# numz/ComfyUI-SeedVR2_VideoUpscaler

Measured on AMD Instinct MI355X. Metric: upscaled frames/sec (720p->4K, SeedVR2-3B), higher is better.
Workload: dtype bf16; 1 GPU; cfg3: SeedVR2-3B 32-frame 720p->4K clip (padded to 33 = 4n+1 for encode + DiT, 32 decoded), VAE tiled 1024/128; vae_tiled=True, parallelism=dp1, weights=random-init SeedVR2-3B + video_vae_v3 architecture (seeded)

## Files before the change

comfyui-seedvr2_videoupscaler_amd/csrc/svr_conv_sub.hip:

```cpp
#include "svr_common.h"
#include "../../include/seedvr2_hip.h"
#include <type_traits>

namespace svr {

constexpr int CS_TY = 16, CS_TX = 32, CS_HX = CS_TX + 1, CS_HY = CS_TY + 1;
constexpr int CS_NT = 256;
constexpr int CS_ROWS = CS_HX * CS_HY;
constexpr int CS_PIECES = (CS_ROWS * 4 + CS_NT - 1) / CS_NT;
constexpr int CS_ABUF = CS_PIECES * CS_NT * 16;
constexpr int CS_NBUF = 4;
constexpr int CS_EP_PITCH = 528;
constexpr int CS_EP_BYTES = 4 * 32 * CS_EP_PITCH;
constexpr int CS_LDS = CS_NBUF * CS_ABUF;
static_assert(CS_PIECES == 9 && CS_EP_BYTES <= CS_LDS, "piece schedule / epilogue parking");

template <int OFF> SVR_DEVICE void cs_rd2(bf16x8 (&r)[2], unsigned a0) {
    const unsigned a1 = a0 ^ 32u;
    asm volatile("ds_read_b128 %0, %2 offset:%4\n\tds_read_b128 %1, %3 offset:%4"
                 : "=&v"(r[0]), "=&v"(r[1]) : "v"(a0), "v"(a1), "n"(OFF) : "memory");
}
template <int N> SVR_DEVICE void cs_wait_rows(bf16x8 (&a)[2]) {
    asm volatile("s_waitcnt lgkmcnt(%2)" : "+v"(a[0]), "+v"(a[1]) : "n"(N));
    __builtin_amdgcn_sched_barrier(0);
}
template <int N> SVR_DEVICE void cs_wait_rows(bf16x8 (&a)[2], bf16x8 (&b)[2]) {
    asm volatile("s_waitcnt lgkmcnt(%4)" : "+v"(a[0]), "+v"(a[1]), "+v"(b[0]), "+v"(b[1]) : "n"(N));
    __builtin_amdgcn_sched_barrier(0);
}
template <int N> SVR_DEVICE void cs_wait_rows(bf16x8 (&a)[2], bf16x8 (&b)[2], bf16x8 (&c)[2], bf16x8 (&d)[2], bf16x8 (&e)[2]) {
    asm volatile("s_waitcnt lgkmcnt(%10)"
                 : "+v"(a[0]), "+v"(a[1]), "+v"(b[0]), "+v"(b[1]), "+v"(c[0]), "+v"(c[1]), "+v"(d[0]), "+v"(d[1]), "+v"(e[0]), "+v"(e[1])
                 : "n"(N));
    __builtin_amdgcn_sched_barrier(0);
}
template <int N> SVR_DEVICE void cs_wait_w(bf16x8 (&w)[2][2]) {
    asm volatile("s_waitcnt vmcnt(%4)" : "+v"(w[0][0]), "+v"(w[0][1]), "+v"(w[1][0]), "+v"(w[1][1]) : "n"(N));
    __builtin_amdgcn_sched_barrier(0);
}

__global__ __launch_bounds__(CS_NT, 1) void conv_sub_kernel(const svr_gemm_args a, const int band_rows) {
    constexpr int MTW = 8, NTW = 2, NT = CS_NT;
    extern __shared__ __attribute__((aligned(16))) char smem[];
    typedef __attribute__((ext_vector_type(16))) float f32x16_t;
    const svr_conv_geom& g = a.conv;
    const int tid = threadIdx.x;
    const int lane = tid & 63;
    const int wave = __builtin_amdgcn_readfirstlane(tid >> 6);
    const int wm = wave >> 1, wn = wave & 1;

    const int tiles_x = (g.W + CS_TX - 1) / CS_TX;
    const int tiles_y = (g.H + CS_TY - 1) / CS_TY;
    const int tiles_n = a.N / 128;
    int tl;
    {
        const int nwg = gridDim.x, bid = blockIdx.x;
        const int xcd = bid & 7, j = bid >> 3, q = nwg >> 3, r = nwg & 7;
        tl = (xcd < r ? xcd * (q + 1) : r * (q + 1) + (xcd - r) * q) + j;
    }
    const bool quad = a.phase.enabled && a.phase.quad != 0;
    int qp = 0;
    if (quad) { qp = tl & 3; tl >>= 2; }
    const int ph_py = quad ? (qp >> 1) : a.phase.py, ph_px = quad ? (qp & 1) : a.phase.px;
    const int pad_h = quad ? 1 - ph_py : g.ph, pad_w = quad ? 1 - ph_px : g.pw;
    const void* const w_frag = quad ? a.phase.W_frag4[qp] : a.W_frag;
    const float* const bias_p = quad ? a.phase.bias4[qp] : a.bias;
    const float* const bias_border_p = quad ? a.phase.bias_border4[qp] : a.phase.bias_border;
    const int tn = tl % tiles_n;
    int rr = tl / tiles_n;
    const int tx = rr % tiles_x; rr /= tiles_x;
    int ty, to;
    if (band_rows > 0 && band_rows < tiles_y) {
        const int per_band = band_rows * g.To;
        const int b = rr / per_band;
        const int rows_b = min(band_rows, tiles_y - b * band_rows);
        const int r2 = rr - b * per_band;
        to = r2 / rows_b;
        ty = b * band_rows + (r2 - to * rows_b);
    } else {
        ty = rr % tiles_y;
        to = rr / tiles_y;
    }
    const int y0 = ty * CS_TY, x0 = tx * CS_TX, n0 = tn * 128;

    const int cpk = g.Cin / 32;
    const int nA = g.kt * cpk;
    const int P = nA * 4;
    const int64_t frame_bytes = (int64_t)g.H * g.W * g.Cin * 2;
    const int srow = tid >> 2, spos = tid & 3;
    uint32_t poff[CS_PIECES];
    uint32_t akeys = 0;
#pragma unroll
    for (int q = 0; q < CS_PIECES; ++q) {
        const int row = q * (NT / 4) + srow;
        const int hy = row / CS_HX, hx = row - hy * CS_HX;
        const int y = y0 - pad_h + hy, x = x0 - pad_w + hx;
        const bool ok = (row < CS_ROWS) & ((unsigned)y < (unsigned)g.H) & ((unsigned)x < (unsigned)g.W);
        poff[q] = ok ? (uint32_t)(y * g.W + x) : 0xffffffffu;
        akeys |= (uint32_t)(spos ^ ((hx >> 2) & 3)) << (2 * q);
    }
    char* const wave_dst = smem + wave * 1024;
    auto frame_ptr = [&](int s) -> const char* {
        if (s >= nA) return nullptr;
        const int dt = s / cpk;
        const int c0 = (s - dt * cpk) * 32;
        int f = to + dt - g.pt;
        const char* basep = (const char*)a.A;
        if (f < 0) {
            if (g.halo != nullptr) { basep = (const char*)g.halo; f += g.halo_frames; }
            else f = 0;
        }
        return basep + (int64_t)f * frame_bytes + c0 * 2;
    };
    auto stage = [&](auto qc, const char* fptr, int buf) {
        constexpr int Q = decltype(qc)::value;
        const int ck = (akeys >> (2 * Q)) & 3;
        const char* src = (poff[Q] == 0xffffffffu || fptr == nullptr) ? (const char*)g.zeros
                                                                      : fptr + ((int64_t)poff[Q] * g.Cin + ck * 8) * 2;
        glds16(src, wave_dst + buf * CS_ABUF + Q * (NT * 16));
    };
    auto stage_all = [&](const char* fptr, int buf) {
        stage(std::integral_constant<int, 0>{}, fptr, buf); stage(std::integral_constant<int, 1>{}, fptr, buf);
        stage(std::integral_constant<int, 2>{}, fptr, buf); stage(std::integral_constant<int, 3>{}, fptr, buf);
        stage(std::integral_constant<int, 4>{}, fptr, buf); stage(std::integral_constant<int, 5>{}, fptr, buf);
        stage(std::integral_constant<int, 6>{}, fptr, buf); stage(std::integral_constant<int, 7>{}, fptr, buf);
        stage(std::integral_constant<int, 8>{}, fptr, buf);
    };

    const int l31 = lane & 31, hi = lane >> 5;
    const unsigned lds0 = (unsigned)(uintptr_t)(__attribute__((address_space(3))) char*)smem;
    unsigned fa[2];
#pragma unroll
    for (int dx = 0; dx < 2; ++dx)
        fa[dx] = lds0 + (unsigned)((wm * MTW * CS_HX + l31) * 64 + ((hi ^ (((dx + l31) >> 2) & 3)) << 4));

    f32x16_t acc[MTW][NTW];
#pragma unroll
    for (int y = 0; y < MTW; ++y)
#pragma unroll
        for (int z = 0; z < NTW; ++z)
#pragma unroll
            for (int e = 0; e < 16; ++e) acc[y][z][e] = 0.f;
    bf16x8 a0[2], a1[2], a2[2], a3[2], a4[2], a5[2], a6[2], a7[2], a8[2];
    bf16x8 w0[NTW][2], w1[NTW][2], w2[NTW][2], w3[NTW][2];

    const int64_t nstride = (int64_t)P * 2048;
    const char* wp0 = (const char*)w_frag + (int64_t)(n0 / 32 + wn * 2) * nstride;
    const char* wp1 = wp0 + nstride;
    const int voff = lane * 16;
    auto wload = [&](bf16x8 (&w)[NTW][2], int k) {
        auto uniform_ptr = [](const char* p) {
            const uint64_t u = (uint64_t)p;
            const uint32_t lo = __builtin_amdgcn_readfirstlane((uint32_t)u), hi_ = __builtin_amdgcn_readfirstlane((uint32_t)(u >> 32));
            return (const char*)(((uint64_t)hi_ << 32) | lo);
        };
        const char* p0 = uniform_ptr(wp0 + (int64_t)min(k, P - 1) * 2048);
        const char* p1 = uniform_ptr(wp1 + (int64_t)min(k, P - 1) * 2048);
        asm volatile("global_load_dwordx4 %0, %1, %2" : "=v"(w[0][0]) : "v"(voff), "s"(p0) : "memory");
        asm volatile("global_load_dwordx4 %0, %1, %2 offset:1024" : "=v"(w[0][1]) : "v"(voff), "s"(p0) : "memory");
        asm volatile("global_load_dwordx4 %0, %1, %2" : "=v"(w[1][0]) : "v"(voff), "s"(p1) : "memory");
        asm volatile("global_load_dwordx4 %0, %1, %2 offset:1024" : "=v"(w[1][1]) : "v"(voff), "s"(p1) : "memory");
    };

#define CS_RD(ROW, R, DXV, BUFOFF) cs_rd2<((R) * CS_HX + (DXV)) * 64>(ROW, fa[DXV] + (BUFOFF))
#define CS_MM(W, KS, ROW, MT, NTI) \
    acc[MT][NTI] = __builtin_amdgcn_mfma_f32_32x32x16_bf16(W[NTI][KS], ROW[KS], acc[MT][NTI], 0, 0, 0)
#define CS_MM8(W, RA, MA, RB, MB) \
    CS_MM(W, 0, RA, MA, 0); CS_MM(W, 0, RA, MA, 1); CS_MM(W, 0, RB, MB, 0); CS_MM(W, 0, RB, MB, 1); \
    CS_MM(W, 1, RA, MA, 0); CS_MM(W, 1, RA, MA, 1); CS_MM(W, 1, RB, MB, 0); CS_MM(W, 1, RB, MB, 1)

    auto interval = [&](auto jc, int s, const char* fstage, bf16x8 (&wc)[NTW][2], bf16x8 (&wn_)[NTW][2]) {
        constexpr int J = decltype(jc)::value;
        constexpr int DX = J >> 1, DY = J & 1;
        constexpr int NPC[4] = {0, 0, 5, 4};
        constexpr int NV = 4 + NPC[(J + 3) & 3] + NPC[(J + 2) & 3];
        const int k = s * 4 + J;
        const unsigned cur = (unsigned)((s & 3) * CS_ABUF), nxt = (unsigned)(((s + 1) & 3) * CS_ABUF);
        const int sbuf = (s + 3) & 3;
        constexpr int NDX = DX ^ 1;
        const unsigned nb = DX == 0 ? cur : nxt;
        if constexpr (DY == 0) {
            CS_RD(a8, 8, DX, cur);
            cs_wait_rows<8>(a0, a1, a2, a3, a4);
            cs_wait_w<NV>(wc);
            CS_MM8(wc, a0, 0, a1, 1);
            __builtin_amdgcn_sched_barrier(0);
            CS_RD(a0, 0, NDX, nb);
            wload(wn_, k + 2);
            __builtin_amdgcn_sched_barrier(0);
            CS_MM8(wc, a2, 2, a3, 3);
            __builtin_amdgcn_sched_barrier(0);
            if constexpr (J == 2) {
                stage(std::integral_constant<int, 0>{}, fstage, sbuf); stage(std::integral_constant<int, 1>{}, fstage, sbuf);
                stage(std::integral_constant<int, 2>{}, fstage, sbuf);
            }
            cs_wait_rows<8>(a4, a5);
            CS_MM8(wc, a4, 4, a5, 5);
            __builtin_amdgcn_sched_barrier(0);
            if constexpr (J == 2) { stage(std::integral_constant<int, 3>{}, fstage, sbuf); stage(std::integral_constant<int, 4>{}, fstage, sbuf); }
            cs_wait_rows<4>(a6, a7);
            CS_MM8(wc, a6, 6, a7, 7);
            __builtin_amdgcn_sched_barrier(0);
        } else {
            cs_wait_w<NV>(wc);
            CS_MM8(wc, a1, 0, a2, 1);
            __builtin_amdgcn_sched_barrier(0);
            CS_RD(a1, 1, NDX, nb); CS_RD(a2, 2, NDX, nb);
            wload(wn_, k + 2);
            __builtin_amdgcn_sched_barrier(0);
            CS_MM8(wc, a3, 2, a4, 3);
            __builtin_amdgcn_sched_barrier(0);
            CS_RD(a3, 3, NDX, nb); CS_RD(a4, 4, NDX, nb);
            if constexpr (J == 3) { stage(std::integral_constant<int, 5>{}, fstage, sbuf); stage(std::integral_constant<int, 6>{}, fstage, sbuf); }
            __builtin_amdgcn_sched_barrier(0);
            CS_MM8(wc, a5, 4, a6, 5);
            __builtin_amdgcn_sched_barrier(0);
            CS_RD(a5, 5, NDX, nb); CS_RD(a6, 6, NDX, nb);
            if constexpr (J == 3) { stage(std::integral_constant<int, 7>{}, fstage, sbuf); stage(std::integral_constant<int, 8>{}, fstage, sbuf); }
            cs_wait_rows<14>(a8);
            CS_MM8(wc, a7, 6, a8, 7);
            __builtin_amdgcn_sched_barrier(0);
            CS_RD(a7, 7, NDX, nb);
            if constexpr (J == 1) {
                __builtin_amdgcn_s_barrier();
                __builtin_amdgcn_sched_barrier(0);
            }
        }
    };

    stage_all(frame_ptr(0), 0);
    stage_all(frame_ptr(1), 1);
    stage_all(frame_ptr(2), 2);
    wload(w0, 0);
    wload(w1, 1);
    __builtin_amdgcn_sched_barrier(0);
#pragma unroll
    for (int y = 0; y < MTW; ++y)
#pragma unroll
        for (int z = 0; z < NTW; ++z) asm volatile("" : "+a"(acc[y][z]));
    asm volatile("s_waitcnt vmcnt(0)" ::: "memory");
    __builtin_amdgcn_s_barrier();
    __builtin_amdgcn_sched_barrier(0);
    CS_RD(a0, 0, 0, 0u); CS_RD(a1, 1, 0, 0u); CS_RD(a2, 2, 0, 0u); CS_RD(a3, 3, 0, 0u);
    CS_RD(a4, 4, 0, 0u); CS_RD(a5, 5, 0, 0u); CS_RD(a6, 6, 0, 0u); CS_RD(a7, 7, 0, 0u);

    for (int s = 0; s < nA; ++s) {
        const char* fs = frame_ptr(s + 3);
        interval(std::integral_constant<int, 0>{}, s, fs, w0, w2);
        interval(std::integral_constant<int, 1>{}, s, fs, w1, w3);
        interval(std::integral_constant<int, 2>{}, s, fs, w2, w0);
        interval(std::integral_constant<int, 3>{}, s, fs, w3, w1);
    }
    asm volatile("s_waitcnt vmcnt(0) lgkmcnt(0)" ::: "memory");
    __builtin_amdgcn_sched_barrier(0);
    __syncthreads();
#undef CS_RD
#undef CS_MM
#undef CS_MM8

    const int hi4 = hi * 4;
    const int n = n0 + (tid & 15) * 8;
    f32x4 bias_lo = {0.f, 0.f, 0.f, 0.f}, bias_hi = {0.f, 0.f, 0.f, 0.f};
    if (bias_p) {
        bias_lo = *(const f32x4*)(bias_p + n);
        bias_hi = *(const f32x4*)(bias_p + n + 4);
    }
    const int py = a.phase.enabled ? ph_py : 0, px = a.phase.enabled ? ph_px : 0;
    const int up = a.phase.enabled ? 2 : 1, ts = a.phase.enabled ? a.phase.t_stride : 1;
    const int yb = py ? g.H - 1 : 0, xb = px ? g.W - 1 : 0;
    const float* btab = a.phase.enabled ? bias_border_p : nullptr;
    double gs0 = 0.0, gq0 = 0.0, gs1 = 0.0, gq1 = 0.0;
    auto ep_body = [&](auto o32c) {
    constexpr int OKIND = decltype(o32c)::value;
    constexpr bool O32 = OKIND == SVR_STORE_FP32;
#pragma unroll
    for (int pass = 0; pass < MTW / 2; ++pass) {
        __builtin_amdgcn_sched_barrier(0);
#pragma unroll
        for (int j = 0; j < 2; ++j) {
            char* row = smem + ((wm * 2 + j) * 32 + l31) * CS_EP_PITCH;
#pragma unroll
            for (int nt = 0; nt < NTW; ++nt) {
                const f32x16_t v = acc[2 * pass + j][nt];
#pragma unroll
                for (int gq = 0; gq < 4; ++gq) {
                    const f32x4 o = {v[4 * gq], v[4 * gq + 1], v[4 * gq + 2], v[4 * gq + 3]};
                    *(f32x4*)(row + (wn * 64 + nt * 32 + 8 * gq + hi4) * 4) = o;
                }
            }
        }
        lds_barrier();
#pragma unroll
        for (int half = 0; half < 2; ++half) {
            f32x4 lo[4], hi_[4];
            int64_t off[4];
            bool ok[4];
            int border[4];
#pragma unroll
            for (int it = 0; it < 4; ++it) {
                const int vox = ((half * 4 + it) * NT + tid) >> 4;
                const int r = vox >> 5;
                const int y = y0 + (r >> 1) * MTW + 2 * pass + (r & 1), x = x0 + (vox & 31);
                ok[it] = y < g.H && x < g.W;
                const int yc = min(y, g.H - 1), xc = min(x, g.W - 1);
                border[it] = (yc == yb ? 1 : 0) | (xc == xb ? 2 : 0);
                off[it] = (((int64_t)to * ts * (up * g.H) + up * yc + py) * (up * g.W) + up * xc + px) * a.N + n;
                lo[it] = *(const f32x4*)(smem + vox * CS_EP_PITCH + (tid & 15) * 32);
                hi_[it] = *(const f32x4*)(smem + vox * CS_EP_PITCH + (tid & 15) * 32 + 16);
            }
#pragma unroll
            for (int it = 0; it < 4; ++it) {
                f32x4 bl = bias_lo, bh = bias_hi;
                if (btab != nullptr && border[it] != 0) {
                    const float* bb = btab + (int64_t)(border[it] - 1) * a.N + n;
                    bl = *(const f32x4*)bb;
                    bh = *(const f32x4*)(bb + 4);
                }
                const float f[8] = {lo[it][0] + bl[0], lo[it][1] + bl[1], lo[it][2] + bl[2], lo[it][3] + bl[3],
                                    hi_[it][0] + bh[0], hi_[it][1] + bh[1], hi_[it][2] + bh[2], hi_[it][3] + bh[3]};
                float r[8];
                if constexpr (O32) {
                    if (ok[it]) {
                        float* cp = (float*)a.C + off[it];
                        *(float4*)cp = make_float4(f[0], f[1], f[2], f[3]);
                        *(float4*)(cp + 4) = make_float4(f[4], f[5], f[6], f[7]);
                    }
#pragma unroll
                    for (int e = 0; e < 8; ++e) r[e] = f[e];
                } else {
                    const uint4 pk = OKIND == SVR_STORE_H16 ? pack8h(f) : pack8(f);
                    if (ok[it]) *(uint4*)((bf16_t*)a.C + off[it]) = pk;
                    if constexpr (OKIND == SVR_STORE_H16) unpack8h(pk, r); else unpack8(pk, r);
                }
                if (a.gn_partial != nullptr && ok[it]) {
                    gn_accumulate4(gs0, gq0, r[0], r[1], r[2], r[3]);
                    gn_accumulate4(gs1, gq1, r[4], r[5], r[6], r[7]);
                }
            }
        }
        if (pass + 1 < MTW / 2) lds_barrier();
    }
    };
    if (a.out_f32 == SVR_STORE_FP32) ep_body(std::integral_constant<int, SVR_STORE_FP32>{});
    else if (a.out_f32 == SVR_STORE_H16) ep_body(std::integral_constant<int, SVR_STORE_H16>{});
    else ep_body(std::integral_constant<int, SVR_STORE_BF16>{});
    if (a.gn_partial) {
        __syncthreads();
        double4* red = (double4*)smem;
        double2* qsum = (double2*)(smem + NT * 32);
        red[tid] = make_double4(gs0, gq0, gs1, gq1);
        __syncthreads();
        if (tid < 32) {
            const int c = tid >> 1, h = tid & 1;
            double s_ = 0.0, q_ = 0.0;
            for (int j = 0; j < NT / 16; ++j) {
                const double4 v = red[(j << 4) | c];
                s_ += h ? v.z : v.x;
                q_ += h ? v.w : v.y;
            }
            qsum[tid] = make_double2(s_, q_);
        }
        __syncthreads();
        const int qpg = (a.N / a.gn_groups) >> 2;
        if (tid < 32 / qpg) {
            double s_ = 0.0, q_ = 0.0;
            for (int i = 0; i < qpg; ++i) { s_ += qsum[tid * qpg + i].x; q_ += qsum[tid * qpg + i].y; }
            const int nblk = tiles_y * tiles_x;
            const int per_frame = a.phase.enabled ? 4 * nblk : nblk;
            const int slot = (a.phase.enabled ? (py * 2 + px) * nblk : 0) + ty * tiles_x + tx;
            ((double2*)a.gn_partial)[((int64_t)to * ts * per_frame + slot) * a.gn_groups + (n0 >> 2) / qpg + tid] = make_double2(s_, q_);
        }
    }
}

int g_conv_sub = 1;

static bool conv_sub_gn_ok(const svr_gemm_args& a) {
    const int cpg = a.gn_groups > 0 ? a.N / a.gn_groups : 0;
    return cpg >= 4 && !(cpg & 3) && a.N % a.gn_groups == 0 && 128 % cpg == 0;
}

static bool conv_sub_eligible(const svr_gemm_args& a) {
    const svr_conv_geom& g = a.conv;
    const bool quad = a.phase.enabled && a.phase.quad != 0;
    bool ptrs = true;
    if (quad) {
        for (int p = 0; p < 4; ++p)
            ptrs = ptrs && a.phase.W_frag4[p] != nullptr && (!a.phase.bias4[p] || ((uintptr_t)a.phase.bias4[p] % 16) == 0) &&
                   (!a.phase.bias_border4[p] || ((uintptr_t)a.phase.bias_border4[p] % 16) == 0);
    } else {
        ptrs = a.W_frag != nullptr && (unsigned)g.ph <= 1u && (unsigned)g.pw <= 1u && (!a.bias || ((uintptr_t)a.bias % 16) == 0) &&
               (!a.phase.bias_border || ((uintptr_t)a.phase.bias_border % 16) == 0);
    }
    return g_conv_sub && g.enabled && ptrs && g.kh == 2 && g.kw == 2 && g.sh == 1 && g.sw == 1 && g.st == 1 &&
           g.Ho == g.H && g.Wo == g.W && g.Cin % 32 == 0 && g.kt >= 1 && g.kt <= 3 &&
           g.To == g.T + g.pt - g.kt + 1 && !a.ps.enabled && a.epilogue == SVR_EPI_BIAS && !a.resid && !a.gate &&
           (!a.gn_partial || conv_sub_gn_ok(a)) && (a.N % 128) == 0 && (a.phase.enabled || (a.ldc == a.N)) &&
           (int64_t)g.H * g.W * g.Cin * 2 < (int64_t)1 << 32 && ((uintptr_t)a.C % 16) == 0;
}

static int conv_sub_gn_blocks(const svr_gemm_args& a) {
    if (!conv_sub_eligible(a) || !conv_sub_gn_ok(a)) return 0;
    const int nblk = ((a.conv.H + CS_TY - 1) / CS_TY) * ((a.conv.W + CS_TX - 1) / CS_TX);
    return a.phase.enabled ? 4 * nblk : nblk;
}

static int launch_conv_sub(const svr_gemm_args& a, hipStream_t s) {
    const svr_conv_geom& g = a.conv;
    const int tiles = g.To * ((g.H + CS_TY - 1) / CS_TY) * ((g.W + CS_TX - 1) / CS_TX) * (a.N / 128) *
                      (a.phase.enabled && a.phase.quad ? 4 : 1);
    static uint64_t lds_attr_done = 0;
    {
        const int e = set_max_dynamic_lds((const void*)conv_sub_kernel, 160 * 1024, lds_attr_done);
        if (e != 0) return e;
    }
    hipLaunchKernelGGL(conv_sub_kernel, dim3(tiles), dim3(CS_NT), CS_LDS, s, a, g_conv_band);
    return (int)hipGetLastError();
}

__global__ __launch_bounds__(256) void conv_pack_frag_taps_kernel(const bf16_t* __restrict__ W, uint4* __restrict__ out, int N, int K,
                                                                  int kt, int kh, int kw, int Cin) {
    const int cpk = Cin / 32, taps = kh * kw, P = kt * cpk * taps;
    const int64_t idx = (int64_t)blockIdx.x * 256 + threadIdx.x;
    if (idx >= (int64_t)(N / 32) * P * 128) return;
    const int lane = (int)(idx & 63), ks = (int)((idx >> 6) & 1);
    const int kk = (int)((idx >> 7) % P), n32 = (int)((idx >> 7) / P);
    const int s = kk / taps, J = kk - s * taps;
    const int dt = s / cpk, cs = s - dt * cpk, dy = J % kh, dx = J / kh;
    const int nn = n32 * 32 + (lane & 31), c = cs * 32 + ks * 16 + (lane >> 5) * 8;
    out[idx] = *(const uint4*)(W + (int64_t)nn * K + ((dt * kh + dy) * kw + dx) * Cin + c);
}

}
```

Measured before the change: 3.703 frames/s.

## Switch conv_sub inner MFMA from 32x32x16 to 16x16x32 bf16 tiles

Replaces each 32x32x16 MFMA with four 16x16x32 MFMAs and rewrites the fragment layout to match: the LDS row addressing and swizzle, the weight-load lane offsets, the accumulator shape, and the epilogue scatter into LDS. The likely aim is the shorter issue latency of the 16x16 instruction and finer interleaving with the LDS reads. In exchange it issues four times as many MFMA instructions for the same work and changes the LDS bank-access pattern.

Measured after the change: 3.728 frames/s (median of 6 runs). No clear change (+0.7%).

```diff
diff --git a/comfyui-seedvr2_videoupscaler_amd/csrc/svr_conv_sub.hip b/comfyui-seedvr2_videoupscaler_amd/csrc/svr_conv_sub.hip
--- a/comfyui-seedvr2_videoupscaler_amd/csrc/svr_conv_sub.hip
+++ b/comfyui-seedvr2_videoupscaler_amd/csrc/svr_conv_sub.hip
@@ -16,9 +16,15 @@
 static_assert(CS_PIECES == 9 && CS_EP_BYTES <= CS_LDS, "piece schedule / epilogue parking");
 
 template <int OFF> SVR_DEVICE void cs_rd2(bf16x8 (&r)[2], unsigned a0) {
-    const unsigned a1 = a0 ^ 32u;
-    asm volatile("ds_read_b128 %0, %2 offset:%4\n\tds_read_b128 %1, %3 offset:%4"
-                 : "=&v"(r[0]), "=&v"(r[1]) : "v"(a0), "v"(a1), "n"(OFF) : "memory");
+    static_assert(OFF >= 0 && OFF + 1024 + 16 <= 65536, "ds_read_b128 offset field");
+    asm volatile("ds_read_b128 %0, %2 offset:%3\n\tds_read_b128 %1, %2 offset:%4"
+                 : "=&v"(r[0]), "=&v"(r[1]) : "v"(a0), "n"(OFF), "n"(OFF + 1024) : "memory");
+}
+SVR_DEVICE void cs_mm4(f32x4 (&c)[2][2], const bf16x8 (&w)[2], const bf16x8 (&r)[2]) {
+    c[0][0] = __builtin_amdgcn_mfma_f32_16x16x32_bf16(w[0], r[0], c[0][0], 0, 0, 0);
+    c[0][1] = __builtin_amdgcn_mfma_f32_16x16x32_bf16(w[1], r[0], c[0][1], 0, 0, 0);
+    c[1][0] = __builtin_amdgcn_mfma_f32_16x16x32_bf16(w[0], r[1], c[1][0], 0, 0, 0);
+    c[1][1] = __builtin_amdgcn_mfma_f32_16x16x32_bf16(w[1], r[1], c[1][1], 0, 0, 0);
 }
 template <int N> SVR_DEVICE void cs_wait_rows(bf16x8 (&a)[2]) {
     asm volatile("s_waitcnt lgkmcnt(%2)" : "+v"(a[0]), "+v"(a[1]) : "n"(N));
@@ -42,7 +48,6 @@
 __global__ __launch_bounds__(CS_NT, 1) void conv_sub_kernel(const svr_gemm_args a, const int band_rows) {
     constexpr int MTW = 8, NTW = 2, NT = CS_NT;
     extern __shared__ __attribute__((aligned(16))) char smem[];
-    typedef __attribute__((ext_vector_type(16))) float f32x16_t;
     const svr_conv_geom& g = a.conv;
     const int tid = threadIdx.x;
     const int lane = tid & 63;
@@ -127,27 +132,27 @@
         stage(std::integral_constant<int, 8>{}, fptr, buf);
     };
 
-    const int l31 = lane & 31, hi = lane >> 5;
+    const int l15 = lane & 15, kq = lane >> 4;
     const unsigned lds0 = (unsigned)(uintptr_t)(__attribute__((address_space(3))) char*)smem;
     unsigned fa[2];
 #pragma unroll
     for (int dx = 0; dx < 2; ++dx)
-        fa[dx] = lds0 + (unsigned)((wm * MTW * CS_HX + l31) * 64 + ((hi ^ (((dx + l31) >> 2) & 3)) << 4));
-
-    f32x16_t acc[MTW][NTW];
+        fa[dx] = lds0 + (unsigned)((wm * MTW * CS_HX + l15) * 64 + ((kq ^ (((dx + l15) >> 2) & 3)) << 4));
+
+    f32x4 acc[MTW][NTW][2][2];
 #pragma unroll
     for (int y = 0; y < MTW; ++y)
 #pragma unroll
         for (int z = 0; z < NTW; ++z)
 #pragma unroll
-            for (int e = 0; e < 16; ++e) acc[y][z][e] = 0.f;
+            for (int e = 0; e < 16; ++e) acc[y][z][e >> 3][(e >> 2) & 1][e & 3] = 0.f;
     bf16x8 a0[2], a1[2], a2[2], a3[2], a4[2], a5[2], a6[2], a7[2], a8[2];
     bf16x8 w0[NTW][2], w1[NTW][2], w2[NTW][2], w3[NTW][2];
 
     const int64_t nstride = (int64_t)P * 2048;
     const char* wp0 = (const char*)w_frag + (int64_t)(n0 / 32 + wn * 2) * nstride;
     const char* wp1 = wp0 + nstride;
-    const int voff = lane * 16;
+    const int voff = kq * 512 + l15 * 16;
     auto wload = [&](bf16x8 (&w)[NTW][2], int k) {
         auto uniform_ptr = [](const char* p) {
             const uint64_t u = (uint64_t)p;
@@ -157,17 +162,14 @@
         const char* p0 = uniform_ptr(wp0 + (int64_t)min(k, P - 1) * 2048);
         const char* p1 = uniform_ptr(wp1 + (int64_t)min(k, P - 1) * 2048);
         asm volatile("global_load_dwordx4 %0, %1, %2" : "=v"(w[0][0]) : "v"(voff), "s"(p0) : "memory");
-        asm volatile("global_load_dwordx4 %0, %1, %2 offset:1024" : "=v"(w[0][1]) : "v"(voff), "s"(p0) : "memory");
+        asm volatile("global_load_dwordx4 %0, %1, %2 offset:256" : "=v"(w[0][1]) : "v"(voff), "s"(p0) : "memory");
         asm volatile("global_load_dwordx4 %0, %1, %2" : "=v"(w[1][0]) : "v"(voff), "s"(p1) : "memory");
-        asm volatile("global_load_dwordx4 %0, %1, %2 offset:1024" : "=v"(w[1][1]) : "v"(voff), "s"(p1) : "memory");
+        asm volatile("global_load_dwordx4 %0, %1, %2 offset:256" : "=v"(w[1][1]) : "v"(voff), "s"(p1) : "memory");
     };
 
 #define CS_RD(ROW, R, DXV, BUFOFF) cs_rd2<((R) * CS_HX + (DXV)) * 64>(ROW, fa[DXV] + (BUFOFF))
-#define CS_MM(W, KS, ROW, MT, NTI) \
-    acc[MT][NTI] = __builtin_amdgcn_mfma_f32_32x32x16_bf16(W[NTI][KS], ROW[KS], acc[MT][NTI], 0, 0, 0)
 #define CS_MM8(W, RA, MA, RB, MB) \
-    CS_MM(W, 0, RA, MA, 0); CS_MM(W, 0, RA, MA, 1); CS_MM(W, 0, RB, MB, 0); CS_MM(W, 0, RB, MB, 1); \
-    CS_MM(W, 1, RA, MA, 0); CS_MM(W, 1, RA, MA, 1); CS_MM(W, 1, RB, MB, 0); CS_MM(W, 1, RB, MB, 1)
+    cs_mm4(acc[MA][0], W[0], RA); cs_mm4(acc[MA][1], W[1], RA); cs_mm4(acc[MB][0], W[0], RB); cs_mm4(acc[MB][1], W[1], RB)
 
     auto interval = [&](auto jc, int s, const char* fstage, bf16x8 (&wc)[NTW][2], bf16x8 (&wn_)[NTW][2]) {
         constexpr int J = decltype(jc)::value;
@@ -237,7 +239,8 @@
 #pragma unroll
     for (int y = 0; y < MTW; ++y)
 #pragma unroll
-        for (int z = 0; z < NTW; ++z) asm volatile("" : "+a"(acc[y][z]));
+        for (int z = 0; z < NTW; ++z)
+            asm volatile("" : "+a"(acc[y][z][0][0]), "+a"(acc[y][z][0][1]), "+a"(acc[y][z][1][0]), "+a"(acc[y][z][1][1]));
     asm volatile("s_waitcnt vmcnt(0)" ::: "memory");
     __builtin_amdgcn_s_barrier();
     __builtin_amdgcn_sched_barrier(0);
@@ -255,10 +258,8 @@
     __builtin_amdgcn_sched_barrier(0);
     __syncthreads();
 #undef CS_RD
-#undef CS_MM
 #undef CS_MM8
 
-    const int hi4 = hi * 4;
     const int n = n0 + (tid & 15) * 8;
     f32x4 bias_lo = {0.f, 0.f, 0.f, 0.f}, bias_hi = {0.f, 0.f, 0.f, 0.f};
     if (bias_p) {
@@ -278,15 +279,14 @@
         __builtin_amdgcn_sched_barrier(0);
 #pragma unroll
         for (int j = 0; j < 2; ++j) {
-            char* row = smem + ((wm * 2 + j) * 32 + l31) * CS_EP_PITCH;
-#pragma unroll
-            for (int nt = 0; nt < NTW; ++nt) {
-                const f32x16_t v = acc[2 * pass + j][nt];
-#pragma unroll
-                for (int gq = 0; gq < 4; ++gq) {
-                    const f32x4 o = {v[4 * gq], v[4 * gq + 1], v[4 * gq + 2], v[4 * gq + 3]};
-                    *(f32x4*)(row + (wn * 64 + nt * 32 + 8 * gq + hi4) * 4) = o;
-                }
+#pragma unroll
+            for (int vh = 0; vh < 2; ++vh) {
+                char* row = smem + ((wm * 2 + j) * 32 + vh * 16 + l15) * CS_EP_PITCH;
+#pragma unroll
+                for (int nt = 0; nt < NTW; ++nt)
+#pragma unroll
+                    for (int ch = 0; ch < 2; ++ch)
+                        *(f32x4*)(row + (wn * 64 + nt * 32 + ch * 16 + kq * 4) * 4) = acc[2 * pass + j][nt][vh][ch];
             }
         }
         lds_barrier();
```
